# tsnorri/vcf2multialign

Measured on AMD Instinct MI355X. Metric: aligned A2M Gbases/sec, higher is better.
Workload: dtype u8

## Files before the change

### vcf2multialign_amd/csrc/kernels.hpp

```cpp
#pragma once

#include <hip/hip_runtime.h>
#include <stdint.h>

#ifdef V2M_CHECKED_BUILD
__device__ uint32_t v2m_lds_poison_seed;
#endif

namespace v2m {

typedef uint32_t u32;
typedef uint64_t u64;

constexpr int kWave = 64;
typedef u32 vec4u __attribute__((ext_vector_type(4)));
typedef vec4u vec4u_unaligned8 __attribute__((aligned(8)));

#ifdef V2M_CHECKED_BUILD
__device__ __forceinline__ u32 poison_hash(u32 seed, u32 wg, u32 i)
{
	u32 h = seed ^ (wg * 0x9E3779B1u) ^ (i * 0x85EBCA77u);
	h ^= h >> 15; h *= 0x2C1B3C6Du;
	h ^= h >> 12; h *= 0x297A2D39u;
	h ^= h >> 15;
// ... 23 lines not shown
}

__global__ __launch_bounds__(256) void poison_fill_kernel(unsigned char *__restrict__ p, u64 n_bytes, u32 seed, u32 salt)
{
	u64 const n_words = n_bytes / 4;
	for (u64 i = (u64) blockIdx.x * 256 + threadIdx.x; i < n_words; i += (u64) gridDim.x * 256)
		reinterpret_cast<u32 *>(p)[i] = poison_hash(seed, salt, (u32) i);
	if (0 == blockIdx.x && threadIdx.x < (n_bytes & 3))
		p[4 * n_words + threadIdx.x] = (unsigned char) (poison_hash(seed, salt, (u32) n_words) >> (8 * threadIdx.x));
}

#define V2M_POISON_LDS(obj) do { ::v2m::poison_lds_object(obj); asm volatile("s_waitcnt lgkmcnt(0)" ::: "memory"); __syncthreads(); } while (0)
#define V2M_POISON_LDS_RANGE(array, begin, end) ::v2m::poison_lds_words(&(array)[0], (begin), (end))
#else
#define V2M_POISON_LDS(obj) ((void) 0)
#define V2M_POISON_LDS_RANGE(array, begin, end) ((void) 0)
#endif

constexpr int kTileBytes = 16384;
constexpr int kSpliceThreads = 256;
constexpr int kTileChunks = kTileBytes / 16;
constexpr int kChunksPerThread = kTileChunks / kSpliceThreads;
constexpr int kLongPatch = 96;

struct __attribute__((aligned(16))) edge_patch {
	u32 aln_begin;
	u32 aln_end;
	u32 label_begin;
	u32 label_len;
};

struct __attribute__((aligned(8))) edge_span {
	u32 src;
	u32 tgt;
};


constexpr int kTrThreads = 256;

__device__ __forceinline__ u64 shfl_xor_u64(u64 v, int mask)
{
	u32 lo = __shfl_xor((u32) v, mask, kWave);
	u32 hi = __shfl_xor((u32) (v >> 32), mask, kWave);
	return ((u64) hi << 32) | lo;
}

// ... 986 lines not shown
				busy &= busy - 1;
				if (lane == j) {
					for (u64 m = w; m; m &= m - 1) {
						int const b = __builtin_ctzll(m);
						edge_span const sp = spans[wi * 64u + b];
						if (sp.src >= c) {
							out |= 1ULL << b;
							c = sp.tgt;
						}
					}
				}
				c = __shfl(c, j, kWave);
			}
			cur = c;
		} else {
			cur = chunk_max > cur ? chunk_max : cur;
		}
		if (wi < word_end)
			eff_row[wi] = out;
	}
}


struct tile_tables {
	u32 const *edge_begin;
	u32 const *cross_offsets;
	u32 const *cross_edges;
};

template <typename LabelPtr>
__device__ __forceinline__ void fill_patch_bytes(
	unsigned char *tile, u32 tile_base, u32 aln_begin, u32 label_len, LabelPtr label,
	u32 from, u32 to, u32 start, u32 step, char gap)
{
	for (u32 pos = from + start; pos < to; pos += step) {
		u32 const off = pos - aln_begin;
		tile[pos - tile_base] = (off < label_len) ? (unsigned char) label[off] : (unsigned char) gap;
	}
}

constexpr int kCandLds = 512;
constexpr int kLabelLds = 1024;
constexpr int kGroupRowsLds = 16;
constexpr int kEffWordsLds = kCandLds / 64 + 2;
constexpr int kLongQueueLds = 16;

struct cached_patch {
	unsigned short begin_rel;
	unsigned short span;
	unsigned short label_rel;
	unsigned short label_len;
};

struct patch_cache {
	cached_patch patch[kCandLds];
	u64 eff[kGroupRowsLds][kEffWordsLds];
	unsigned char labels[kLabelLds];
	u32 long_queue[kLongQueueLds];
	u32 long_count;
};

struct tile_job {
	u32 tile_base, tile_end;
	u32 cross_begin, n_cross, range_begin, n_range;
	u32 n_lds;
	u32 w0;
};

__device__ __forceinline__ void load_eff_cache(
	patch_cache &pc, tile_job const &job, u64 const *__restrict__ eff, u64 eff_words_per_row, u32 first_row, u32 n_rows, int t)
{
	if (0 == job.n_lds) return;
	u32 const nw = ((job.range_begin + job.n_lds - 1) >> 6) - job.w0 + 1;
	u32 const rows = n_rows < (u32) kGroupRowsLds ? n_rows : (u32) kGroupRowsLds;
	for (u32 i = t; i < rows * nw; i += kSpliceThreads)
		pc.eff[i / nw][i % nw] = eff[(u64) (first_row + i / nw) * eff_words_per_row + job.w0 + i % nw];
}

template <bool kWindow = false>
__device__ __forceinline__ void load_patch_cache(
	patch_cache &pc, tile_job &job, tile_tables const &tt, edge_patch const *__restrict__ patches, char const *__restrict__ labels,
	u64 const *__restrict__ eff, u64 eff_words_per_row, u32 tile, u32 row_begin, u32 n_group_rows, int t, u32 col_base = 0, u32 col_end = 0)
{
	job.tile_base = (kWindow ? col_base : 0u) + tile * (u32) kTileBytes;
	job.tile_end = (kWindow && col_end - job.tile_base < (u32) kTileBytes) ? col_end : job.tile_base + kTileBytes;
	job.cross_begin = tt.cross_offsets[tile];
	job.n_cross = tt.cross_offsets[tile + 1] - job.cross_begin;
	job.range_begin = tt.edge_begin[tile];
	job.n_range = tt.edge_begin[tile + 1] - job.range_begin;
	job.n_lds = job.n_range < (u32) kCandLds ? job.n_range : (u32) kCandLds;
	job.w0 = job.range_begin >> 6;
	if (job.n_lds) {
		u32 const label_base = patches[job.range_begin].label_begin;
		for (u32 i = t; i < job.n_lds; i += kSpliceThreads) {
			edge_patch const p = patches[job.range_begin + i];
			u32 const span = p.aln_end - p.aln_begin, rel = p.label_begin - label_base;
			cached_patch c;
			c.begin_rel = (unsigned short) (p.aln_begin - job.tile_base);
			c.span = span < 0xFFFFu ? (unsigned short) span : (unsigned short) 0xFFFF;
			bool const label_ok = rel + p.label_len <= (u32) kLabelLds;
			c.label_rel = label_ok ? (unsigned short) rel : (unsigned short) 0xFFFF;
			c.label_len = label_ok ? (unsigned short) p.label_len : (unsigned short) 0;
			pc.patch[i] = c;
		}
		edge_patch const last = patches[job.range_begin + job.n_lds - 1];
		u32 const label_span = last.label_begin + last.label_len - label_base;
		u32 const label_len = label_span < (u32) kLabelLds ? label_span : (u32) kLabelLds;
		for (u32 i = t; i < label_len; i += kSpliceThreads)
			pc.labels[i] = (unsigned char) labels[label_base + i];
	}
	load_eff_cache(pc, job, eff, eff_words_per_row, row_begin, n_group_rows, t);
	if (t == 0) pc.long_count = 0;
}

struct tile_patch {
	u32 edge;
	u32 aln_begin;
	u32 from, to;
	u32 label_len;
	u32 label_begin;
	bool in_lds;
};

__device__ __forceinline__ u32 candidate_edge(tile_job const &job, tile_tables const &tt, u32 i)
{
	return (i < job.n_cross) ? tt.cross_edges[job.cross_begin + i] : job.range_begin + (i - job.n_cross);
}

__device__ __forceinline__ bool candidate_in_lds(tile_job const &job, u32 i)
{
	return i >= job.n_cross && i - job.n_cross < job.n_lds;
}

template <bool kWindow = false>
// ... 76 lines not shown
	if (n_long) {
		for (u32 q = t >> 6; q < n_long; q += kSpliceThreads >> 6) {
			edge_patch const p = patches[pc.long_queue[q]];
			u32 const from = p.aln_begin > job.tile_base ? p.aln_begin : job.tile_base;
			u32 const to = p.aln_end < tile_end ? p.aln_end : tile_end;
			fill_patch_bytes(buf, job.tile_base, p.aln_begin, p.label_len, labels + p.label_begin, from, to, t & 63, 64, gap);
		}
		__syncthreads();
		if (t == 0) pc.long_count = 0;
	}
	V2M_POISON_LDS_RANGE(pc.long_queue, 0u, (u32) kLongQueueLds);
}

__device__ __forceinline__ void map_block(u32 b, u32 n_groups, u32 n_tiles, u32 tile_run, u32 &tile, u32 &group)
{
	u32 const per_super = tile_run * n_groups;
	u32 const super = b / per_super, within = b % per_super;
	u32 const t0 = super * tile_run;
	u32 const run = (n_tiles - t0 < tile_run) ? n_tiles - t0 : tile_run;
	group = within / run;
	tile = t0 + within % run;
}

template <bool kNonTemporal, bool kWindow>
__device__ __forceinline__ void splice_aligned_tiles(
	vec4u const *__restrict__ tmpl, u64 const *__restrict__ eff, u64 eff_words_per_row,
	tile_tables tt, edge_patch const *__restrict__ patches, char const *__restrict__ labels,
	char *__restrict__ out, u64 row_pitch, u32 n_rows, u32 rows_per_group, u32 n_groups, u32 n_tiles, u32 tile_run,
	u64 store_limit, char gap, u32 col_base, u32 col_end)
{
	__shared__ vec4u lds[2][kTileChunks];
	__shared__ patch_cache pc;

	int const t = threadIdx.x;
	u32 tile, group;
	map_block(blockIdx.x, n_groups, n_tiles, tile_run, tile, group);
	u32 const row_begin = group * rows_per_group;
	u32 const row_end = (row_begin + rows_per_group < n_rows) ? row_begin + rows_per_group : n_rows;
	V2M_POISON_LDS(lds);
	V2M_POISON_LDS(pc);

	vec4u pristine[kChunksPerThread];
#pragma unroll
	for (int k = 0; k < kChunksPerThread; ++k)
		pristine[k] = tmpl[(u64) tile * kTileChunks + t + kSpliceThreads * k];

	tile_job job;
	load_patch_cache<kWindow>(pc, job, tt, patches, labels, eff, eff_words_per_row, tile, row_begin, row_end - row_begin, t, col_base, col_end);
	u32 const tile_base = job.tile_base;

	for (u32 row = row_begin; row < row_end; ++row) {
		vec4u *const buf = lds[(row - row_begin) & 1];
		u32 const cached_row = (row - row_begin) % (u32) kGroupRowsLds;
		if (row != row_begin && 0 == cached_row)
			load_eff_cache(pc, job, eff, eff_words_per_row, row, row_end - row, t);
#pragma unroll
		for (int k = 0; k < kChunksPerThread; ++k)
			buf[t + kSpliceThreads * k] = pristine[k];
		__syncthreads();

		patch_row_tile<kWindow>((unsigned char *) buf, pc, job, tt, patches, labels, eff + (u64) row * eff_words_per_row, cached_row, t, gap);

		char *const dst = out + (u64) row * row_pitch + (u64) tile * kTileBytes;
#pragma unroll
		for (int k = 0; k < kChunksPerThread; ++k) {
			int const c = t + kSpliceThreads * k;
			if ((kWindow ? (u64) tile * kTileBytes : (u64) tile_base) + (u64) c * 16 < store_limit) {
				vec4u const nv = buf[c];
				if (kNonTemporal)
					__builtin_nontemporal_store(nv, (vec4u *) (dst + c * 16));
				else
					*(vec4u *) (dst + c * 16) = nv;
			}
		}
	}
}

template <bool kNonTemporal>
__global__ __launch_bounds__(kSpliceThreads) void splice_aligned_kernel(
	vec4u const *__restrict__ tmpl, u64 const *__restrict__ eff, u64 eff_words_per_row,
	tile_tables tt, edge_patch const *__restrict__ patches, char const *__restrict__ labels,
	char *__restrict__ out, u64 row_pitch, u32 n_rows, u32 rows_per_group, u32 n_groups, u32 n_tiles, u32 tile_run,
	u64 store_limit , char gap)
{
	splice_aligned_tiles<kNonTemporal, false>(tmpl, eff, eff_words_per_row, tt, patches, labels, out, row_pitch, n_rows, rows_per_group, n_groups,
		n_tiles, tile_run, store_limit, gap, 0u, 0u);
}

template <bool kNonTemporal>
__global__ __launch_bounds__(kSpliceThreads) void splice_aligned_window_kernel(
	vec4u const *__restrict__ tmpl, u64 const *__restrict__ eff, u64 eff_words_per_row,
	tile_tables tt, edge_patch const *__restrict__ patches, char const *__restrict__ labels,
	char *__restrict__ out, u64 row_pitch, u32 n_rows, u32 rows_per_group, u32 n_groups, u32 n_tiles, u32 tile_run,
	u64 store_limit, char gap, u32 col_base, u32 col_end)
{
	splice_aligned_tiles<kNonTemporal, true>(tmpl, eff, eff_words_per_row, tt, patches, labels, out, row_pitch, n_rows, rows_per_group, n_groups,
		n_tiles, tile_run, store_limit, gap, col_base, col_end);
}


__device__ __forceinline__ u32 zero_bytes_mask(u32 x)
{
	return ~(((x & 0x7F7F7F7Fu) + 0x7F7F7F7Fu) | x | 0x7F7F7F7Fu);
}

__device__ __forceinline__ u32 wave_inclusive_scan_u32(u32 v)
{
	v += (u32) __builtin_amdgcn_update_dpp(0, (int) v, 0x111, 0xf, 0xf, false);
	v += (u32) __builtin_amdgcn_update_dpp(0, (int) v, 0x112, 0xf, 0xf, false);
	v += (u32) __builtin_amdgcn_update_dpp(0, (int) v, 0x114, 0xf, 0xf, false);
	v += (u32) __builtin_amdgcn_update_dpp(0, (int) v, 0x118, 0xf, 0xf, false);
	v += (u32) __builtin_amdgcn_update_dpp(0, (int) v, 0x142, 0xa, 0xf, false);
	v += (u32) __builtin_amdgcn_update_dpp(0, (int) v, 0x143, 0xc, 0xf, false);
	return v;
}

template <int kN>
__device__ __forceinline__ void wave_inclusive_scan_u32_lockstep(u32 (&v)[kN])
{
// ... 484 lines not shown
	__syncthreads();
	for (u32 base = 0; base < n_tiles; base += 256) {
		u32 const i = base + t;
		u32 const mine = i < n_tiles ? row[i] : 0;
		u32 const incl = wave_inclusive_scan_u32(mine);
		if (lane == 63) wave_sums[wave] = incl;
		__syncthreads();
		u32 before = carry_s, total = 0;
#pragma unroll
		for (int wv = 0; wv < 4; ++wv) {
			u32 const ws = wave_sums[wv];
			if (wv < wave) before += ws;
			total += ws;
		}
		if (i < n_tiles) row[i] = before + incl - mine;
		__syncthreads();
		if (t == 0) carry_s += total;
		__syncthreads();
	}
	if (t == 0) row_lengths[blockIdx.x] = carry_s;
}


__global__ __launch_bounds__(kSpliceThreads) void probe_write_kernel(char *__restrict__ out, u64 pitch, u32 n_groups)
{
	u32 const tile = blockIdx.x / n_groups, group = blockIdx.x % n_groups;
	vec4u const v = {0, 0, 0, 0};
	for (u32 r = 0; r < 16; ++r) {
		char *const dst = out + (u64) (group * 16 + r) * pitch + (u64) tile * kTileBytes;
#pragma unroll
		for (int k = 0; k < kChunksPerThread; ++k)
			__builtin_nontemporal_store(v, (vec4u *) (dst + (threadIdx.x + kSpliceThreads * k) * 16));
	}
}


__host__ __device__ __forceinline__ u64 mix64(u64 z)
{
	z ^= z >> 30; z *= 0xBF58476D1CE4E5B9ULL;
	z ^= z >> 27; z *= 0x94D049BB133111EBULL;
	z ^= z >> 31;
	return z;
}

constexpr u64 kGolden = 0x9E3779B97F4A7C15ULL;

__global__ __launch_bounds__(256) void checksum_rows_kernel(
	char const *__restrict__ rows, u64 row_pitch, u64 const *__restrict__ lengths, u64 fixed_length,
	u64 words_per_block, unsigned long long *__restrict__ sums)
{
	u32 const row = blockIdx.y;
	u64 const len = lengths ? lengths[row] : fixed_length;
	u64 const n_words = (len + 7) / 8;
	u64 const w_begin = (u64) blockIdx.x * words_per_block;
	u64 w_end = w_begin + words_per_block;
// ... 22 lines not shown
```

### vcf2multialign_amd/csrc/v2m_hip.hip

```cpp

#include <hip/hip_runtime.h>

#include <algorithm>
#include <atomic>
#include <chrono>
#include <condition_variable>
#include <cstdarg>
#include <cstdio>
#include <cstdlib>
#include <cstring>
#include <memory>
#include <mutex>
#include <string>
#include <thread>
#include <utility>
#include <vector>

#include <type_traits>

#include "../../include/v2m_hip.h"
#include "kernels.hpp"
#include "founder_kernels.hpp"
#include "bgzf_kernels.hpp"

// ... 100 lines not shown


struct held_ring_state {
	std::mutex mutex;
	std::condition_variable released;
};

struct v2m_row_hold {
	pinned_buf host;
	hipEvent_t copied{};
	uint64_t outstanding{};
	held_ring_state *ring{};
};


struct word_range { u64 restart, lo, hi, stride; };

struct row_view {
	u64 begin{}, end{};
	u64 max_unaligned{};
	u32 n_tiles{};
	dev_buf d_template, d_template0;
	bool has_template0{};
	dev_buf d_edge_begin, d_cross_offsets, d_cross_edges;
	word_range words{};
	u64 length() const { return end - begin; }
};


struct v2m_ctx {
	int device{};
	u32 n_cus{256};
	hipStream_t stream{};
	hipStream_t copy_stream{};
	std::string err;

	bool profiling{};
	std::vector<event_pair> events[V2M_KERNEL_COUNT];
	std::vector<event_pair> free_events;

	bool has_graph{};
	u64 n_nodes{}, n_edges{}, ref_len{}, aligned_len{}, label_bytes{};
	bool has_nul_byte{};
	std::vector<u32> h_csum;
	std::vector<u32> h_tgt_prefix_max;
	dev_buf d_ref, d_ref_pos, d_aln_pos, d_spans, d_patches, d_labels, d_overlappable;
	dev_buf d_ovl_rank, d_blocker_masks;
	std::vector<u32> h_aln_pos, h_tile_edge_begin, h_cross_offsets, h_cross_edges;
// ... 71 lines not shown
	{
		if (!ctx->profiling) return;
		if (!ctx->free_events.empty()) { ev = ctx->free_events.back(); ctx->free_events.pop_back(); }
		else if (hipSuccess != hipEventCreate(&ev.begin) || hipSuccess != hipEventCreate(&ev.end)) return;
		active = (hipSuccess == hipEventRecord(ev.begin, ctx->stream));
	}
	~timed_launch()
	{
		if (!active) return;
		(void) hipEventRecord(ev.end, ctx->stream);
		ctx->events[kernel].push_back(ev);
	}
};


template <typename T>
int upload_vec(v2m_ctx *ctx, dev_buf &dst, std::vector<T> const &src, size_t min_bytes = 16)
{
	size_t const bytes(std::max(src.size() * sizeof(T), min_bytes));
	V2M_HIP_TRY(ctx, dst.ensure(bytes));
	if (!src.empty())
		V2M_HIP_TRY(ctx, hipMemcpyAsync(dst.p, src.data(), src.size() * sizeof(T), hipMemcpyHostToDevice, ctx->stream));
	return V2M_OK;
}


struct scoped_events {
	std::vector<hipEvent_t> ev;
	~scoped_events() { for (auto e : ev) (void) hipEventDestroy(e); }
	hipError_t create(std::size_t n)
	{
		for (std::size_t i(0); i < n; ++i) {
			hipEvent_t e{};
			hipError_t const st(hipEventCreate(&e));
			if (hipSuccess != st) return st;
			ev.push_back(e);
		}
		return hipSuccess;
	}
	hipEvent_t operator[](std::size_t i) const { return ev[i]; }
};

struct scoped_profiling_off {
	v2m_ctx *ctx;
	bool was;
	explicit scoped_profiling_off(v2m_ctx *c) : ctx(c), was(c->profiling) { c->profiling = false; }
// ... 380 lines not shown
			out.seg_copy[n] = copy;
			++n;
			prev = node;
		}
	});
	std::vector<row_error> errors(n_rows);
	unsigned const n_threads(out.n_segments >= (u64(1) << 20) ? unsigned(std::min<u64>(n_rows, 8)) : 1u);
	if (n_threads <= 1) {
		for (u64 r(row_begin); r < row_end; ++r) { fill_row(r, errors[r - row_begin]); if (V2M_OK != errors[r - row_begin].code) break; }
	}
	else {
		std::atomic<u64> next(row_begin);
		auto const work([&] { for (u64 r; (r = next.fetch_add(1)) < row_end;) fill_row(r, errors[r - row_begin]); });
		std::vector<std::thread> pool;
		for (unsigned t(1); t < n_threads; ++t) pool.emplace_back(work);
		work();
		for (auto &t : pool) t.join();
	}
	for (auto const &e : errors) if (V2M_OK != e.code) return fail(ctx, e.code, "%s", e.text.c_str());
	return V2M_OK;
}


int forced_store_mode(bool unaligned)
{
	if (unaligned) {
		char const *const e = std::getenv("V2M_UNALIGNED_STORE");
		if (e && 0 == std::strcmp(e, "plain")) return 0;
		if (e && 0 == std::strcmp(e, "nt")) return 1;
		return -1;
	}
	char const *e = std::getenv("V2M_NT_STORES");
	if (!(e && *e)) return -1;
	return std::atoi(e) != 0 ? 1 : 0;
}

u32 rows_per_group_for(u64 n_rows)
{
	char const *e = std::getenv("V2M_ROWS_PER_GROUP");
	int const v((e && *e) ? std::atoi(e) : 0);
	if (v > 0) return u32(std::min(v, 256));
	return u32(std::min<u64>(32, std::max<u64>(1, n_rows)));
}


int expand_reference(v2m_ctx *ctx, row_view const &v, dev_buf &dst, char gap)
{
	u64 const n_chunks(u64(v.n_tiles) * v2m::kTileChunks);
	V2M_HIP_TRY(ctx, dst.ensure(n_chunks * 16));
	{
		timed_launch tl(ctx, V2M_KERNEL_TEMPLATE);
		hipLaunchKernelGGL(v2m::expand_reference_row_kernel, dim3(unsigned((n_chunks + 255) / 256)), dim3(256), 0, ctx->stream,
			ctx->d_ref.as<char>(), ctx->d_ref_pos.as<u32>(), ctx->d_aln_pos.as<u32>(), u32(ctx->n_nodes), u32(v.end), n_chunks, dst.as<uint4>(), gap, u32(v.begin));
	}
// ... 80 lines not shown
	u64 n_blocks;
};

u32 tile_run_for(u32 n_tiles)
{
	char const *e = std::getenv("V2M_TILE_RUN");
	int const v((e && *e) ? std::atoi(e) : 0);
	u32 const run(v > 0 ? u32(v) : 64u);
	return std::max<u32>(1, std::min(run, n_tiles));
}

int make_grid(v2m_ctx *ctx, u64 n_rows, splice_grid &g)
{
	g.rows_per_group = rows_per_group_for(n_rows);
	g.n_groups = u32((n_rows + g.rows_per_group - 1) / g.rows_per_group);
	g.n_blocks = u64(ctx->view().n_tiles) * g.n_groups;
	g.tile_run = tile_run_for(ctx->view().n_tiles);
	if (g.n_blocks > 0x7FFFFFFFull)
		return fail(ctx, V2M_ERR_UNSUPPORTED, "splice grid too large (%llu workgroups); use smaller batches", (unsigned long long) g.n_blocks);
	return V2M_OK;
}


template <typename F>
int store_flavour_launch(v2m_ctx *ctx, bool unaligned, u64 n_rows, u64 bytes, F const &launch)
{
	int &slot(unaligned ? ctx->unaligned_store_mode : ctx->store_mode);
	int mode(forced_store_mode(unaligned));
	if (mode < 0) mode = slot;
	if (mode < 0 && bytes >= (u64(1) << 30)) {
		scoped_events ev;
		V2M_HIP_TRY(ctx, ev.create(5));
		V2M_HIP_TRY(ctx, hipEventRecord(ev[0], ctx->stream));
		for (int i(0); i < 4; ++i) {
			launch(0 == (i & 1));
			V2M_HIP_TRY(ctx, hipEventRecord(ev[i + 1], ctx->stream));
		}
		V2M_HIP_TRY(ctx, hipStreamSynchronize(ctx->stream));
		float t[4];
		for (int i(0); i < 4; ++i) V2M_HIP_TRY(ctx, hipEventElapsedTime(&t[i], ev[i], ev[i + 1]));
		float const nt_ms(std::min(t[0], t[2])), plain_ms(std::min(t[1], t[3]));
		slot = nt_ms <= plain_ms ? 1 : 0;
		char buf[160];
		std::snprintf(buf, sizeof(buf), "%s splice stores: %s (calibrated on %llu rows: nontemporal %.3f ms, plain %.3f ms)",
			unaligned ? "unaligned" : "aligned", slot ? "nontemporal" : "plain", (unsigned long long) n_rows, nt_ms, plain_ms);
		if (unaligned && ctx->info.size() > 2000) ctx->info.clear();
		if (!ctx->info.empty()) ctx->info += "; ";
		ctx->info += buf;
		mode = slot;
	}
	if (mode < 0) mode = 1;
	{
		timed_launch tl(ctx, unaligned ? V2M_KERNEL_SPLICE_UNALIGNED : V2M_KERNEL_SPLICE_ALIGNED);
		launch(0 != mode);
	}
	V2M_HIP_TRY(ctx, hipGetLastError());
	return V2M_OK;
}


int splice_aligned_slice(v2m_ctx *ctx, v2m_row_batch const *rows, u64 row_begin, u64 row_end, char *d_out, u64 row_pitch)
{
	u64 const n_rows(row_end - row_begin);
	if (0 == n_rows || 0 == ctx->aligned_len) return V2M_OK;
	if (int const rc = resolve_slice(ctx, rows, row_begin, row_end)) return rc;

	row_view const &v(ctx->view());
	splice_grid g;
	if (int const rc = make_grid(ctx, n_rows, g)) return rc;
	v2m::tile_tables const tt{v.d_edge_begin.as<u32>(), v.d_cross_offsets.as<u32>(), v.d_cross_edges.as<u32>()};
	u64 const store_limit((v.length() + 15) & ~u64(15));
	auto const launch([&](bool nt) {
		auto const go([&](auto kernel, auto... window) {
			hipLaunchKernelGGL(kernel, dim3(unsigned(g.n_blocks)), dim3(v2m::kSpliceThreads), 0, ctx->stream,
				v.d_template.as<v2m::vec4u>(), ctx->d_eff.as<u64>() - v.words.restart, v.words.stride, tt, ctx->d_patches.as<v2m::edge_patch>(), ctx->d_labels.as<char>(),
				d_out, row_pitch, u32(n_rows), g.rows_per_group, g.n_groups, v.n_tiles, g.tile_run, store_limit, '-', window...);
		});
		if (ctx->windowed) {
			if (nt) go(v2m::splice_aligned_window_kernel<true>, u32(v.begin), u32(v.end));
			else go(v2m::splice_aligned_window_kernel<false>, u32(v.begin), u32(v.end));
		}
		else if (nt) go(v2m::splice_aligned_kernel<true>);
		else go(v2m::splice_aligned_kernel<false>);
	});
	return store_flavour_launch(ctx, false, n_rows, n_rows * v.length(), launch);
}


int splice_unaligned_slice(v2m_ctx *ctx, v2m_row_batch const *rows, u64 row_begin, u64 row_end, char *d_out, u64 row_pitch)
{
	u64 const n_rows(row_end - row_begin);
	if (0 == n_rows) return V2M_OK;
	V2M_HIP_TRY(ctx, ctx->d_row_lengths.ensure(n_rows * sizeof(u64)));
	if (0 == ctx->aligned_len) {
		V2M_HIP_TRY(ctx, hipMemsetAsync(ctx->d_row_lengths.p, 0, n_rows * sizeof(u64), ctx->stream));
		return V2M_OK;
	}
	row_view &v(ctx->view());
	if (!v.has_template0) {
		if (int const rc = expand_reference(ctx, v, v.d_template0, 0)) return rc;
		v.has_template0 = true;
	}
	if (int const rc = resolve_slice(ctx, rows, row_begin, row_end)) return rc;

	splice_grid g;
	if (int const rc = make_grid(ctx, n_rows, g)) return rc;
	V2M_HIP_TRY(ctx, ctx->d_tile_counts.ensure(n_rows * v.n_tiles * sizeof(u32)));
	bool const windowed(ctx->windowed);
	v2m::tile_tables const tt{v.d_edge_begin.as<u32>(), v.d_cross_offsets.as<u32>(), v.d_cross_edges.as<u32>()};
	u64 const *const d_eff(ctx->d_eff.as<u64>() - v.words.restart);
	{
		char const *const ce(std::getenv("V2M_COUNT_ROWS_PER_GROUP"));
		u32 const count_rows(u32(std::min<u64>(std::max<u64>(1, n_rows), (ce && *ce && std::atoi(ce) > 0) ? u64(std::min(std::atoi(ce), int(v2m::kCountRowsMax))) : u64(v2m::kCountRowsMax))));
		u32 const count_groups(u32((n_rows + count_rows - 1) / count_rows));
		timed_launch tl(ctx, V2M_KERNEL_UNALIGNED_COUNT);
		auto const count([&](auto kernel, auto... window) {
			hipLaunchKernelGGL(kernel, dim3(unsigned(u64(v.n_tiles) * count_groups)), dim3(v2m::kSpliceThreads), 0, ctx->stream,
				v.d_template0.as<v2m::vec4u>(), d_eff, v.words.stride, tt, ctx->d_patches.as<v2m::edge_patch>(), ctx->d_labels.as<char>(),
				ctx->d_tile_counts.as<u32>(), v.n_tiles, u32(n_rows), count_rows, count_groups, g.tile_run, window...);
		});
		if (windowed) count(v2m::count_unaligned_window_kernel, u32(v.begin), u32(v.end));
		else count(v2m::count_unaligned_kernel);
		hipLaunchKernelGGL(v2m::scan_tile_counts_kernel, dim3(unsigned(n_rows)), dim3(256), 0, ctx->stream,
			ctx->d_tile_counts.as<u32>(), v.n_tiles, ctx->d_row_lengths.as<u64>());
	}
	auto const launch([&](bool nt) {
		auto const go([&](auto kernel, auto... window) {
			hipLaunchKernelGGL(kernel, dim3(unsigned(g.n_blocks)), dim3(v2m::kSpliceThreads), 0, ctx->stream,
				v.d_template0.as<v2m::vec4u>(), d_eff, v.words.stride, tt, ctx->d_patches.as<v2m::edge_patch>(), ctx->d_labels.as<char>(),
				ctx->d_tile_counts.as<u32>(), v.n_tiles, d_out, row_pitch, u32(n_rows), g.rows_per_group, g.n_groups, g.tile_run, window...);
		});
		if (windowed) {
			if (nt) go(v2m::splice_unaligned_window_kernel<true>, u32(v.begin), u32(v.end));
			else go(v2m::splice_unaligned_window_kernel<false>, u32(v.begin), u32(v.end));
			return;
		}
#ifdef V2M_TUNING_BUILD
		static int const flavour([] { char const *const e(std::getenv("V2M_UNALIGNED_KERNEL")); return !e ? 0 : 0 == std::strcmp(e, "wave") ? 1 : 0 == std::strcmp(e, "shared64") ? 2 : 0; }());
		if (1 == flavour) { if (nt) go(v2m::splice_unaligned_per_wave_kernel<true>); else go(v2m::splice_unaligned_per_wave_kernel<false>); return; }
		if (2 == flavour) { if (nt) go(v2m::splice_unaligned_kernel<true, 64>); else go(v2m::splice_unaligned_kernel<false, 64>); return; }
#endif
		if (nt) go(v2m::splice_unaligned_kernel<true>);
		else go(v2m::splice_unaligned_kernel<false>);
	});
	return store_flavour_launch(ctx, true, n_rows, n_rows * (windowed ? v.length() : ctx->ref_len), launch);
}


int check_batch(v2m_ctx *ctx, v2m_row_batch const *rows, u32 flags)
{
	if (!ctx) return V2M_ERR_INVALID_ARGUMENT;
	if (!rows) return fail(ctx, V2M_ERR_INVALID_ARGUMENT, "rows is NULL");
	if (flags & ~(V2M_SPLICE_UNALIGNED | V2M_SPLICE_BGZF)) return fail(ctx, V2M_ERR_INVALID_ARGUMENT, "unknown flags 0x%x", flags);
	if (!ctx->has_graph) return fail(ctx, V2M_ERR_STATE, "no graph uploaded");
	if (rows->n_rows && !rows->copy_index && !rows->cut_offsets) return fail(ctx, V2M_ERR_INVALID_ARGUMENT, "rows->copy_index is NULL");
	if (rows->cut_offsets && rows->cut_offsets[rows->n_rows] && (!rows->cut_nodes || !rows->cut_copies))
		return fail(ctx, V2M_ERR_INVALID_ARGUMENT, "cut arrays are NULL");
	if (rows->n_rows >= 0xFFFFFFFFull) return fail(ctx, V2M_ERR_UNSUPPORTED, "too many rows in one batch");
	if (ctx->d_by_edge.p) { ctx->d_by_edge.reset(); ctx->by_edge_valid = false; }
	if ((flags & V2M_SPLICE_UNALIGNED) && ctx->has_nul_byte)
		return fail(ctx, V2M_ERR_UNSUPPORTED, "the reference sequence or an ALT label holds a NUL byte, which the unaligned kernels use as their padding marker; aligned mode keeps such bytes");
	return V2M_OK;
}


struct slice_plan { u64 pitch, rows_per_slice, n_slices, slot_bytes; };

slice_plan plan_slices(v2m_ctx const *ctx, u64 n_rows, bool unaligned, u64 max_rows_per_slice = ~u64(0))
// ... 601 lines not shown
	ctx->n_nodes = N; ctx->n_edges = E; ctx->ref_len = ref_len; ctx->aligned_len = L; ctx->label_bytes = label_total;
	V2M_HIP_TRY(ctx, ctx->d_ref.ensure(std::max<u64>(ref_len, 16)));
	if (ref_len) V2M_HIP_TRY(ctx, hipMemcpyAsync(ctx->d_ref.p, ref_seq, ref_len, hipMemcpyHostToDevice, ctx->stream));
	V2M_HIP_TRY(ctx, ctx->d_labels.ensure(std::max<u64>(label_total, 16)));
	if (label_total) V2M_HIP_TRY(ctx, hipMemcpyAsync(ctx->d_labels.p, g->alt_edge_label_bytes, label_total, hipMemcpyHostToDevice, ctx->stream));
	if (int const rc = upload_vec(ctx, ctx->d_ref_pos, ref_pos)) return rc;
	if (int const rc = upload_vec(ctx, ctx->d_aln_pos, aln_pos)) return rc;
	if (int const rc = upload_vec(ctx, ctx->d_spans, spans)) return rc;
	if (int const rc = upload_vec(ctx, ctx->d_patches, patches)) return rc;
	if (int const rc = upload_vec(ctx, ctx->d_overlappable, overlappable)) return rc;
	if (int const rc = upload_vec(ctx, ctx->d_ovl_rank, ovl_rank)) return rc;
	if (int const rc = upload_vec(ctx, ctx->d_blocker_masks, blocker_masks)) return rc;

	row_view &v(ctx->whole);
	v.begin = 0;
	v.end = L;
	v.max_unaligned = ref_len + label_total;
	v.n_tiles = n_tiles;
	v.has_template0 = false;
	v.words = {0, 0, (E + 63) / 64, (((E + 63) / 64) + 15) & ~u64(15)};
	if (int const rc = upload_vec(ctx, v.d_edge_begin, tile_edge_begin)) return rc;
	if (int const rc = upload_vec(ctx, v.d_cross_offsets, cross_offsets)) return rc;
	if (int const rc = upload_vec(ctx, v.d_cross_edges, cross_edges)) return rc;
	if (int const rc = expand_reference(ctx, v, v.d_template, '-')) return rc;

	ctx->d_paths = nullptr;
	ctx->by_edge_valid = false;
	ctx->path_rows = ctx->path_cols = ctx->path_pitch = 0;
	if (g->paths_by_chrom_copy_and_edge) {
		size_t const bytes(g->path_rows / 64 * g->path_cols * sizeof(u64));
		V2M_HIP_TRY(ctx, ctx->owned_paths.ensure(std::max<size_t>(bytes, 16)));
		if (bytes) V2M_HIP_TRY(ctx, hipMemcpyAsync(ctx->owned_paths.p, g->paths_by_chrom_copy_and_edge, bytes, hipMemcpyHostToDevice, ctx->stream));
		ctx->d_paths = ctx->owned_paths.as<u64>();
		ctx->path_rows = g->path_rows;
		ctx->path_cols = g->path_cols;
		ctx->path_pitch = g->path_rows / 64;
	}
	V2M_HIP_TRY(ctx, hipStreamSynchronize(ctx->stream));

	ctx->has_nul_byte = (ref_len && std::memchr(ref_seq, 0, ref_len)) || (label_total && std::memchr(g->alt_edge_label_bytes, 0, label_total));
	ctx->h_csum = std::move(csum);
	ctx->h_tgt_prefix_max = std::move(tgt_prefix_max);
	ctx->h_aln_pos = std::move(aln_pos);
	ctx->h_patches = std::move(patches);
	ctx->h_overlappable = std::move(overlappable);
	ctx->h_tile_edge_begin = std::move(tile_edge_begin);
// ... 171 lines not shown
	u32 const e_hi(edge_begin[n_tiles]);
	u64 e_lo(0), hi(e_hi);
	while (e_lo < hi) {
		u64 const mid((e_lo + hi) / 2);
		if (ctx->h_aln_pos[ctx->h_tgt_prefix_max[mid + 1]] > col_begin) hi = mid; else e_lo = mid + 1;
	}
	row_view &w(ctx->window);
	u64 restart(0), lo(0), word_hi(0);
	if (e_lo < e_hi) {
		lo = e_lo / 64;
		word_hi = (u64(e_hi) + 63) / 64;
		restart = lo;
		while (restart > 0 && (ctx->h_overlappable[restart] & 1)) --restart;
	}
	w.words = {restart, lo, word_hi, (word_hi - restart + 15) & ~u64(15)};
	w.begin = col_begin;
	w.end = col_end;
	w.max_unaligned = W;
	w.n_tiles = n_tiles;
	w.has_template0 = false;
	if (int const rc = upload_vec(ctx, w.d_edge_begin, edge_begin)) return rc;
	if (int const rc = upload_vec(ctx, w.d_cross_offsets, cross_offsets)) return rc;
	if (int const rc = upload_vec(ctx, w.d_cross_edges, cross_edges)) return rc;
	if (int const rc = expand_reference(ctx, w, w.d_template, '-')) return rc;
	V2M_HIP_TRY(ctx, hipStreamSynchronize(ctx->stream));
	ctx->windowed = true;
	return V2M_OK;
}



namespace {

int pbwt_check_state(v2m_ctx *ctx, uint64_t n_copies, uint64_t n_chunks, const uint32_t *start_order, int max_copies)
{
	if (0 == n_copies || n_copies > u64(max_copies)) return fail(ctx, V2M_ERR_UNSUPPORTED, "this GPU chunk walk holds at most %d chromosome copies (got %llu)", max_copies, (unsigned long long) n_copies);
	if (n_copies > ctx->path_cols) return fail(ctx, V2M_ERR_INVALID_ARGUMENT, "the bound path matrix has %llu copies, %llu asked for", (unsigned long long) ctx->path_cols, (unsigned long long) n_copies);
	if (ctx->path_cols > u64(max_copies)) return fail(ctx, V2M_ERR_UNSUPPORTED, "this GPU chunk walk reads edge columns of at most %d copies; the bound path matrix has %llu columns", max_copies, (unsigned long long) ctx->path_cols);
	if (ctx->n_edges >= 0x7FFFFFF0ull) return fail(ctx, V2M_ERR_UNSUPPORTED, "the GPU chunk walk keeps edge indices in 31 bits (the graph has %llu edges)", (unsigned long long) ctx->n_edges);
	for (u64 i(0), n(n_chunks * n_copies); i < n; ++i)
		if (start_order[i] >= n_copies) return fail(ctx, V2M_ERR_INVALID_ARGUMENT, "start_order[%llu] = %u is not a chromosome copy (%llu copies)", (unsigned long long) i, start_order[i], (unsigned long long) n_copies);
	return V2M_OK;
}

int edge_major_paths(v2m_ctx *ctx, u64 const **d_by_edge_out)
{
// ... 291 lines not shown
	});
}

void v2m_row_release(v2m_row_hold *hold)
{
	if (!hold) return;
	std::lock_guard<std::mutex> const lock(hold->ring->mutex);
	if (hold->outstanding && 0 == --hold->outstanding) hold->ring->released.notify_all();
}




namespace {

int probe_output(v2m_ctx *ctx, void *p, u64 pitch, u32 n_groups, float &ms_out)
{
	scoped_events ev;
	V2M_HIP_TRY(ctx, ev.create(2));
	u32 const n_tiles(u32(pitch / v2m::kTileBytes));
	ms_out = 1e30f;
	for (int rep(0); rep < 3; ++rep) {
		V2M_HIP_TRY(ctx, hipEventRecord(ev[0], ctx->stream));
		hipLaunchKernelGGL(v2m::probe_write_kernel, dim3(n_tiles * n_groups), dim3(v2m::kSpliceThreads), 0, ctx->stream, static_cast<char *>(p), pitch, n_groups);
		V2M_HIP_TRY(ctx, hipEventRecord(ev[1], ctx->stream));
		V2M_HIP_TRY(ctx, hipEventSynchronize(ev[1]));
		float t(0);
		V2M_HIP_TRY(ctx, hipEventElapsedTime(&t, ev[0], ev[1]));
		if (rep) ms_out = std::min(ms_out, t);
	}
	return V2M_OK;
}

}

int v2m_alloc_output(v2m_ctx *ctx, uint64_t bytes, int candidates, void **d_out)
{
	if (!ctx) return V2M_ERR_INVALID_ARGUMENT;
	if (!d_out || 0 == bytes) return fail(ctx, V2M_ERR_INVALID_ARGUMENT, "bad v2m_alloc_output arguments");
	*d_out = nullptr;
	V2M_HIP_TRY(ctx, hipSetDevice(ctx->device));

	u32 const n_groups(32);
	u64 const pitch((bytes / (n_groups * 16)) & ~u64(v2m::kTileBytes - 1));
	bool const can_probe(pitch >= u64(64) * v2m::kTileBytes);
	auto const note([&](std::string const &text) {
		if (ctx->info.size() > 2000) ctx->info.clear();
// ... 375 lines not shown
```

Baseline: 6874.

## Use buffer stores with cache-policy flavours and precomputed tile descriptors in aligned splice

Aligned splice stores now go through raw buffer stores with selectable cache-policy bits (nt, sc1_nt, sc0_sc1_nt, plain), and the runtime calibration picks the fastest of these flavours. The buffer resource range replaces the per-chunk store_limit bounds check. Per-tile metadata and label extents are precomputed on the host into a tile_desc array, so the patch, label and eff-cache loads are issued up front as unrolled buffer loads. The eff cache refill is moved after patching, which overlaps it with the stores. This adds a host-side table and a wider calibration sweep over large outputs. It relies on out-of-range buffer accesses being dropped.

Measured after the change: 6850, median of 2. No clear change (-0.3%).

```diff
diff --git a/vcf2multialign_amd/csrc/kernels.hpp b/vcf2multialign_amd/csrc/kernels.hpp
--- a/vcf2multialign_amd/csrc/kernels.hpp
+++ b/vcf2multialign_amd/csrc/kernels.hpp
@@ -69,6 +69,26 @@
 constexpr int kTileChunks = kTileBytes / 16;
 constexpr int kChunksPerThread = kTileChunks / kSpliceThreads;
 constexpr int kLongPatch = 96;
+
+enum class store_flavour : int { plain = 0, nt = 1, sc1 = 2, sc1_nt = 3, sc0_sc1 = 4, sc0_sc1_nt = 5, flat_nt = 6 };
+
+__host__ __device__ constexpr int store_aux(store_flavour f)
+{
+	return store_flavour::nt == f ? 2 : store_flavour::sc1 == f ? 16 : store_flavour::sc1_nt == f ? 18
+		: store_flavour::sc0_sc1 == f ? 17 : store_flavour::sc0_sc1_nt == f ? 19 : 0;
+}
+
+__device__ __forceinline__ __amdgpu_buffer_rsrc_t tile_store_rsrc(char *p, u32 bytes)
+{
+	return __builtin_amdgcn_make_buffer_rsrc(p,  0, (int) bytes, 0x00020000);
+}
+
+template <store_flavour kFlavour>
+__device__ __forceinline__ void store_tile_chunk(__amdgpu_buffer_rsrc_t rsrc, u32 off, u32 __attribute__((ext_vector_type(4))) value)
+{
+	static_assert(store_flavour::flat_nt != kFlavour, "flat_nt is not a buffer store");
+	__builtin_amdgcn_raw_buffer_store_b128(value, rsrc, (int) off, 0, store_aux(kFlavour));
+}
 
 struct __attribute__((aligned(16))) edge_patch {
 	u32 aln_begin;
@@ -1101,10 +1121,12 @@
 }
 
 
+struct tile_desc;
 struct tile_tables {
 	u32 const *edge_begin;
 	u32 const *cross_offsets;
 	u32 const *cross_edges;
+	tile_desc const *desc;
 };
 
 template <typename LabelPtr>
@@ -1139,6 +1161,13 @@
 	u32 long_count;
 };
 
+struct __attribute__((aligned(32))) tile_desc {
+	u32 range_begin, n_range;
+	u32 cross_begin, n_cross;
+	u32 label_base, label_bytes;
+	u32 reserved[2];
+};
+
 struct tile_job {
 	u32 tile_base, tile_end;
 	u32 cross_begin, n_cross, range_begin, n_range;
@@ -1163,32 +1192,53 @@
 {
 	job.tile_base = (kWindow ? col_base : 0u) + tile * (u32) kTileBytes;
 	job.tile_end = (kWindow && col_end - job.tile_base < (u32) kTileBytes) ? col_end : job.tile_base + kTileBytes;
-	job.cross_begin = tt.cross_offsets[tile];
-	job.n_cross = tt.cross_offsets[tile + 1] - job.cross_begin;
-	job.range_begin = tt.edge_begin[tile];
-	job.n_range = tt.edge_begin[tile + 1] - job.range_begin;
+	tile_desc const d = tt.desc[tile];
+	job.cross_begin = d.cross_begin;
+	job.n_cross = d.n_cross;
+	job.range_begin = d.range_begin;
+	job.n_range = d.n_range;
 	job.n_lds = job.n_range < (u32) kCandLds ? job.n_range : (u32) kCandLds;
 	job.w0 = job.range_begin >> 6;
-	if (job.n_lds) {
-		u32 const label_base = patches[job.range_begin].label_begin;
-		for (u32 i = t; i < job.n_lds; i += kSpliceThreads) {
-			edge_patch const p = patches[job.range_begin + i];
-			u32 const span = p.aln_end - p.aln_begin, rel = p.label_begin - label_base;
-			cached_patch c;
-			c.begin_rel = (unsigned short) (p.aln_begin - job.tile_base);
-			c.span = span < 0xFFFFu ? (unsigned short) span : (unsigned short) 0xFFFF;
-			bool const label_ok = rel + p.label_len <= (u32) kLabelLds;
-			c.label_rel = label_ok ? (unsigned short) rel : (unsigned short) 0xFFFF;
-			c.label_len = label_ok ? (unsigned short) p.label_len : (unsigned short) 0;
-			pc.patch[i] = c;
-		}
-		edge_patch const last = patches[job.range_begin + job.n_lds - 1];
-		u32 const label_span = last.label_begin + last.label_len - label_base;
-		u32 const label_len = label_span < (u32) kLabelLds ? label_span : (u32) kLabelLds;
-		for (u32 i = t; i < label_len; i += kSpliceThreads)
-			pc.labels[i] = (unsigned char) labels[label_base + i];
-	}
-	load_eff_cache(pc, job, eff, eff_words_per_row, row_begin, n_group_rows, t);
+
+	constexpr int kPatchLoads = kCandLds / kSpliceThreads, kLabelLoads = kLabelLds / kSpliceThreads;
+	static_assert(kPatchLoads * kSpliceThreads == kCandLds && kLabelLoads * kSpliceThreads == kLabelLds, "whole rounds of the workgroup");
+	static_assert(kGroupRowsLds * kEffWordsLds <= kSpliceThreads, "one effective-edge word per thread");
+	__amdgpu_buffer_rsrc_t const patch_rsrc = __builtin_amdgcn_make_buffer_rsrc(
+		const_cast<edge_patch *>(patches + job.range_begin), 0, (int) (job.n_lds * (u32) sizeof(edge_patch)), 0x00020000);
+	__amdgpu_buffer_rsrc_t const label_rsrc = __builtin_amdgcn_make_buffer_rsrc(const_cast<char *>(labels + d.label_base), 0, (int) d.label_bytes, 0x00020000);
+	vec4u pv[kPatchLoads];
+	unsigned char lb[kLabelLoads];
+#pragma unroll
+	for (int k = 0; k < kPatchLoads; ++k)
+		pv[k] = __builtin_amdgcn_raw_buffer_load_b128(patch_rsrc, (int) ((t + kSpliceThreads * k) * sizeof(edge_patch)), 0, 0);
+#pragma unroll
+	for (int k = 0; k < kLabelLoads; ++k)
+		lb[k] = __builtin_amdgcn_raw_buffer_load_b8(label_rsrc, t + kSpliceThreads * k, 0, 0);
+	u32 const nw = job.n_lds ? ((job.range_begin + job.n_lds - 1) >> 6) - job.w0 + 1 : 0u;
+	u32 const eff_rows = n_group_rows < (u32) kGroupRowsLds ? n_group_rows : (u32) kGroupRowsLds;
+	bool const has_eff = (u32) t < eff_rows * nw;
+	u32 const eff_r = has_eff ? (u32) t / nw : 0u, eff_w = has_eff ? (u32) t % nw : 0u;
+	u64 eff_word = 0;
+	if (has_eff) eff_word = eff[(u64) (row_begin + eff_r) * eff_words_per_row + job.w0 + eff_w];
+
+#pragma unroll
+	for (int k = 0; k < kPatchLoads; ++k) {
+		u32 const i = t + kSpliceThreads * k;
+		if (i >= job.n_lds) continue;
+		edge_patch const p{pv[k].x, pv[k].y, pv[k].z, pv[k].w};
+		u32 const span = p.aln_end - p.aln_begin, rel = p.label_begin - d.label_base;
+		cached_patch c;
+		c.begin_rel = (unsigned short) (p.aln_begin - job.tile_base);
+		c.span = span < 0xFFFFu ? (unsigned short) span : (unsigned short) 0xFFFF;
+		bool const label_ok = rel + p.label_len <= (u32) kLabelLds;
+		c.label_rel = label_ok ? (unsigned short) rel : (unsigned short) 0xFFFF;
+		c.label_len = label_ok ? (unsigned short) p.label_len : (unsigned short) 0;
+		pc.patch[i] = c;
+	}
+#pragma unroll
+	for (int k = 0; k < kLabelLoads; ++k)
+		if ((u32) (t + kSpliceThreads * k) < d.label_bytes) pc.labels[t + kSpliceThreads * k] = lb[k];
+	if (has_eff) pc.eff[eff_r][eff_w] = eff_word;
 	if (t == 0) pc.long_count = 0;
 }
 
@@ -1311,7 +1361,7 @@
 	tile = t0 + within % run;
 }
 
-template <bool kNonTemporal, bool kWindow>
+template <store_flavour kFlavour, bool kWindow>
 __device__ __forceinline__ void splice_aligned_tiles(
 	vec4u const *__restrict__ tmpl, u64 const *__restrict__ eff, u64 eff_words_per_row,
 	tile_tables tt, edge_patch const *__restrict__ patches, char const *__restrict__ labels,
@@ -1336,13 +1386,12 @@
 
 	tile_job job;
 	load_patch_cache<kWindow>(pc, job, tt, patches, labels, eff, eff_words_per_row, tile, row_begin, row_end - row_begin, t, col_base, col_end);
-	u32 const tile_base = job.tile_base;
+	u64 const tile_off = (u64) tile * kTileBytes;
+	u32 const tile_bytes = store_limit <= tile_off ? 0u : store_limit - tile_off < (u64) kTileBytes ? (u32) (store_limit - tile_off) : (u32) kTileBytes;
 
 	for (u32 row = row_begin; row < row_end; ++row) {
 		vec4u *const buf = lds[(row - row_begin) & 1];
 		u32 const cached_row = (row - row_begin) % (u32) kGroupRowsLds;
-		if (row != row_begin && 0 == cached_row)
-			load_eff_cache(pc, job, eff, eff_words_per_row, row, row_end - row, t);
 #pragma unroll
 		for (int k = 0; k < kChunksPerThread; ++k)
 			buf[t + kSpliceThreads * k] = pristine[k];
@@ -1350,40 +1399,37 @@
 
 		patch_row_tile<kWindow>((unsigned char *) buf, pc, job, tt, patches, labels, eff + (u64) row * eff_words_per_row, cached_row, t, gap);
 
-		char *const dst = out + (u64) row * row_pitch + (u64) tile * kTileBytes;
+		if (cached_row + 1 == (u32) kGroupRowsLds && row + 1 < row_end)
+			load_eff_cache(pc, job, eff, eff_words_per_row, row + 1, row_end - (row + 1), t);
+
+		__amdgpu_buffer_rsrc_t const rsrc = tile_store_rsrc(out + (u64) row * row_pitch + tile_off, tile_bytes);
 #pragma unroll
 		for (int k = 0; k < kChunksPerThread; ++k) {
 			int const c = t + kSpliceThreads * k;
-			if ((kWindow ? (u64) tile * kTileBytes : (u64) tile_base) + (u64) c * 16 < store_limit) {
-				vec4u const nv = buf[c];
-				if (kNonTemporal)
-					__builtin_nontemporal_store(nv, (vec4u *) (dst + c * 16));
-				else
-					*(vec4u *) (dst + c * 16) = nv;
-			}
-		}
-	}
-}
-
-template <bool kNonTemporal>
+			store_tile_chunk<kFlavour>(rsrc, (u32) c * 16, buf[c]);
+		}
+	}
+}
+
+template <store_flavour kFlavour>
 __global__ __launch_bounds__(kSpliceThreads) void splice_aligned_kernel(
 	vec4u const *__restrict__ tmpl, u64 const *__restrict__ eff, u64 eff_words_per_row,
 	tile_tables tt, edge_patch const *__restrict__ patches, char const *__restrict__ labels,
 	char *__restrict__ out, u64 row_pitch, u32 n_rows, u32 rows_per_group, u32 n_groups, u32 n_tiles, u32 tile_run,
 	u64 store_limit , char gap)
 {
-	splice_aligned_tiles<kNonTemporal, false>(tmpl, eff, eff_words_per_row, tt, patches, labels, out, row_pitch, n_rows, rows_per_group, n_groups,
+	splice_aligned_tiles<kFlavour, false>(tmpl, eff, eff_words_per_row, tt, patches, labels, out, row_pitch, n_rows, rows_per_group, n_groups,
 		n_tiles, tile_run, store_limit, gap, 0u, 0u);
 }
 
-template <bool kNonTemporal>
+template <store_flavour kFlavour>
 __global__ __launch_bounds__(kSpliceThreads) void splice_aligned_window_kernel(
 	vec4u const *__restrict__ tmpl, u64 const *__restrict__ eff, u64 eff_words_per_row,
 	tile_tables tt, edge_patch const *__restrict__ patches, char const *__restrict__ labels,
 	char *__restrict__ out, u64 row_pitch, u32 n_rows, u32 rows_per_group, u32 n_groups, u32 n_tiles, u32 tile_run,
 	u64 store_limit, char gap, u32 col_base, u32 col_end)
 {
-	splice_aligned_tiles<kNonTemporal, true>(tmpl, eff, eff_words_per_row, tt, patches, labels, out, row_pitch, n_rows, rows_per_group, n_groups,
+	splice_aligned_tiles<kFlavour, true>(tmpl, eff, eff_words_per_row, tt, patches, labels, out, row_pitch, n_rows, rows_per_group, n_groups,
 		n_tiles, tile_run, store_limit, gap, col_base, col_end);
 }
 
@@ -1914,15 +1960,23 @@
 }
 
 
-__global__ __launch_bounds__(kSpliceThreads) void probe_write_kernel(char *__restrict__ out, u64 pitch, u32 n_groups)
+template <store_flavour kFlavour>
+__global__ __launch_bounds__(kSpliceThreads) void probe_write_kernel(char *__restrict__ out, u64 pitch, u32 n_groups, u32 fill)
 {
 	u32 const tile = blockIdx.x / n_groups, group = blockIdx.x % n_groups;
-	vec4u const v = {0, 0, 0, 0};
+	vec4u const v = {fill, fill * (threadIdx.x | 1u), fill * (tile | 1u), fill ^ (fill >> 7)};
 	for (u32 r = 0; r < 16; ++r) {
 		char *const dst = out + (u64) (group * 16 + r) * pitch + (u64) tile * kTileBytes;
-#pragma unroll
-		for (int k = 0; k < kChunksPerThread; ++k)
-			__builtin_nontemporal_store(v, (vec4u *) (dst + (threadIdx.x + kSpliceThreads * k) * 16));
+		if constexpr (store_flavour::flat_nt == kFlavour) {
+#pragma unroll
+			for (int k = 0; k < kChunksPerThread; ++k)
+				__builtin_nontemporal_store(v, (vec4u *) (dst + (threadIdx.x + kSpliceThreads * k) * 16));
+		} else {
+			__amdgpu_buffer_rsrc_t const rsrc = tile_store_rsrc(dst, (u32) kTileBytes);
+#pragma unroll
+			for (int k = 0; k < kChunksPerThread; ++k)
+				store_tile_chunk<kFlavour>(rsrc, (threadIdx.x + kSpliceThreads * k) * 16u, v);
+		}
 	}
 }
 
diff --git a/vcf2multialign_amd/csrc/v2m_hip.hip b/vcf2multialign_amd/csrc/v2m_hip.hip
--- a/vcf2multialign_amd/csrc/v2m_hip.hip
+++ b/vcf2multialign_amd/csrc/v2m_hip.hip
@@ -146,8 +146,9 @@
 	u32 n_tiles{};
 	dev_buf d_template, d_template0;
 	bool has_template0{};
-	dev_buf d_edge_begin, d_cross_offsets, d_cross_edges;
+	dev_buf d_edge_begin, d_cross_offsets, d_cross_edges, d_tile_desc;
 	word_range words{};
+	v2m::tile_tables tables() const { return {d_edge_begin.as<u32>(), d_cross_offsets.as<u32>(), d_cross_edges.as<u32>(), d_tile_desc.as<v2m::tile_desc>()}; }
 	u64 length() const { return end - begin; }
 };
 
@@ -265,6 +266,22 @@
 	if (!src.empty())
 		V2M_HIP_TRY(ctx, hipMemcpyAsync(dst.p, src.data(), src.size() * sizeof(T), hipMemcpyHostToDevice, ctx->stream));
 	return V2M_OK;
+}
+
+
+std::vector<v2m::tile_desc> make_tile_descs(std::vector<v2m::edge_patch> const &patches, std::vector<u32> const &edge_begin, std::vector<u32> const &cross_offsets, u32 n_tiles)
+{
+	std::vector<v2m::tile_desc> descs(n_tiles);
+	for (u32 t(0); t < n_tiles; ++t) {
+		v2m::tile_desc &d(descs[t]);
+		d = {edge_begin[t], edge_begin[t + 1] - edge_begin[t], cross_offsets[t], cross_offsets[t + 1] - cross_offsets[t], 0, 0, {0, 0}};
+		u32 const n_lds(std::min<u32>(d.n_range, v2m::kCandLds));
+		if (!n_lds) continue;
+		v2m::edge_patch const &last(patches[d.range_begin + n_lds - 1]);
+		d.label_base = patches[d.range_begin].label_begin;
+		d.label_bytes = std::min<u32>(last.label_begin + last.label_len - d.label_base, v2m::kLabelLds);
+	}
+	return descs;
 }
 
 
@@ -691,6 +708,12 @@
 }
 
 
+struct flavour_name { int mode; char const *name; };
+constexpr flavour_name kUnalignedFlavours[] = {{1, "nontemporal"}, {0, "plain"}};
+constexpr flavour_name kAlignedFlavours[] = {
+	{int(v2m::store_flavour::nt), "nt"}, {int(v2m::store_flavour::sc1_nt), "sc1_nt"},
+	{int(v2m::store_flavour::sc0_sc1_nt), "sc0_sc1_nt"}, {int(v2m::store_flavour::plain), "plain"}};
+
 int forced_store_mode(bool unaligned)
 {
 	if (unaligned) {
@@ -699,6 +722,9 @@
 		if (e && 0 == std::strcmp(e, "nt")) return 1;
 		return -1;
 	}
+	if (char const *const name = std::getenv("V2M_ALIGNED_STORE"))
+		for (auto const &f : kAlignedFlavours)
+			if (0 == std::strcmp(name, f.name)) return f.mode;
 	char const *e = std::getenv("V2M_NT_STORES");
 	if (!(e && *e)) return -1;
 	return std::atoi(e) != 0 ? 1 : 0;
@@ -825,37 +851,48 @@
 }
 
 
-template <typename F>
-int store_flavour_launch(v2m_ctx *ctx, bool unaligned, u64 n_rows, u64 bytes, F const &launch)
+template <std::size_t kN, typename F>
+int store_flavour_launch(v2m_ctx *ctx, bool unaligned, flavour_name const (&flavours)[kN], u64 n_rows, u64 bytes, F const &launch)
 {
 	int &slot(unaligned ? ctx->unaligned_store_mode : ctx->store_mode);
 	int mode(forced_store_mode(unaligned));
 	if (mode < 0) mode = slot;
 	if (mode < 0 && bytes >= (u64(1) << 30)) {
 		scoped_events ev;
-		V2M_HIP_TRY(ctx, ev.create(5));
+		V2M_HIP_TRY(ctx, ev.create(2 * kN + 1));
 		V2M_HIP_TRY(ctx, hipEventRecord(ev[0], ctx->stream));
-		for (int i(0); i < 4; ++i) {
-			launch(0 == (i & 1));
+		for (std::size_t i(0); i < 2 * kN; ++i) {
+			launch(flavours[i % kN].mode);
 			V2M_HIP_TRY(ctx, hipEventRecord(ev[i + 1], ctx->stream));
 		}
 		V2M_HIP_TRY(ctx, hipStreamSynchronize(ctx->stream));
-		float t[4];
-		for (int i(0); i < 4; ++i) V2M_HIP_TRY(ctx, hipEventElapsedTime(&t[i], ev[i], ev[i + 1]));
-		float const nt_ms(std::min(t[0], t[2])), plain_ms(std::min(t[1], t[3]));
-		slot = nt_ms <= plain_ms ? 1 : 0;
-		char buf[160];
-		std::snprintf(buf, sizeof(buf), "%s splice stores: %s (calibrated on %llu rows: nontemporal %.3f ms, plain %.3f ms)",
-			unaligned ? "unaligned" : "aligned", slot ? "nontemporal" : "plain", (unsigned long long) n_rows, nt_ms, plain_ms);
+		float ms[kN];
+		std::size_t best(0);
+		for (std::size_t i(0); i < kN; ++i) {
+			float a(0), b(0);
+			V2M_HIP_TRY(ctx, hipEventElapsedTime(&a, ev[i], ev[i + 1]));
+			V2M_HIP_TRY(ctx, hipEventElapsedTime(&b, ev[kN + i], ev[kN + i + 1]));
+			ms[i] = std::min(a, b);
+			if (ms[i] < ms[best]) best = i;
+		}
+		slot = flavours[best].mode;
+		char buf[96];
+		std::snprintf(buf, sizeof(buf), "%s splice stores: %s (calibrated on %llu rows:", unaligned ? "unaligned" : "aligned", flavours[best].name, (unsigned long long) n_rows);
+		std::string text(buf);
+		for (std::size_t i(0); i < kN; ++i) {
+			std::snprintf(buf, sizeof(buf), "%s %s %.3f ms", i ? "," : "", flavours[i].name, ms[i]);
+			text += buf;
+		}
+		text += ")";
 		if (unaligned && ctx->info.size() > 2000) ctx->info.clear();
 		if (!ctx->info.empty()) ctx->info += "; ";
-		ctx->info += buf;
+		ctx->info += text;
 		mode = slot;
 	}
 	if (mode < 0) mode = 1;
 	{
 		timed_launch tl(ctx, unaligned ? V2M_KERNEL_SPLICE_UNALIGNED : V2M_KERNEL_SPLICE_ALIGNED);
-		launch(0 != mode);
+		launch(mode);
 	}
 	V2M_HIP_TRY(ctx, hipGetLastError());
 	return V2M_OK;
@@ -871,22 +908,28 @@
 	row_view const &v(ctx->view());
 	splice_grid g;
 	if (int const rc = make_grid(ctx, n_rows, g)) return rc;
-	v2m::tile_tables const tt{v.d_edge_begin.as<u32>(), v.d_cross_offsets.as<u32>(), v.d_cross_edges.as<u32>()};
+	v2m::tile_tables const tt(v.tables());
 	u64 const store_limit((v.length() + 15) & ~u64(15));
-	auto const launch([&](bool nt) {
+	auto const launch([&](int mode) {
 		auto const go([&](auto kernel, auto... window) {
 			hipLaunchKernelGGL(kernel, dim3(unsigned(g.n_blocks)), dim3(v2m::kSpliceThreads), 0, ctx->stream,
 				v.d_template.as<v2m::vec4u>(), ctx->d_eff.as<u64>() - v.words.restart, v.words.stride, tt, ctx->d_patches.as<v2m::edge_patch>(), ctx->d_labels.as<char>(),
 				d_out, row_pitch, u32(n_rows), g.rows_per_group, g.n_groups, v.n_tiles, g.tile_run, store_limit, '-', window...);
 		});
-		if (ctx->windowed) {
-			if (nt) go(v2m::splice_aligned_window_kernel<true>, u32(v.begin), u32(v.end));
-			else go(v2m::splice_aligned_window_kernel<false>, u32(v.begin), u32(v.end));
-		}
-		else if (nt) go(v2m::splice_aligned_kernel<true>);
-		else go(v2m::splice_aligned_kernel<false>);
+		auto const with([&](auto flavour) {
+			constexpr v2m::store_flavour kF(decltype(flavour)::value);
+			if (ctx->windowed) go(v2m::splice_aligned_window_kernel<kF>, u32(v.begin), u32(v.end));
+			else go(v2m::splice_aligned_kernel<kF>);
+		});
+		using sf = v2m::store_flavour;
+		switch (sf(mode)) {
+			case sf::plain: with(std::integral_constant<sf, sf::plain>{}); break;
+			case sf::sc1_nt: with(std::integral_constant<sf, sf::sc1_nt>{}); break;
+			case sf::sc0_sc1_nt: with(std::integral_constant<sf, sf::sc0_sc1_nt>{}); break;
+			default: with(std::integral_constant<sf, sf::nt>{}); break;
+		}
 	});
-	return store_flavour_launch(ctx, false, n_rows, n_rows * v.length(), launch);
+	return store_flavour_launch(ctx, false, kAlignedFlavours, n_rows, n_rows * v.length(), launch);
 }
 
 
@@ -910,7 +953,7 @@
 	if (int const rc = make_grid(ctx, n_rows, g)) return rc;
 	V2M_HIP_TRY(ctx, ctx->d_tile_counts.ensure(n_rows * v.n_tiles * sizeof(u32)));
 	bool const windowed(ctx->windowed);
-	v2m::tile_tables const tt{v.d_edge_begin.as<u32>(), v.d_cross_offsets.as<u32>(), v.d_cross_edges.as<u32>()};
+	v2m::tile_tables const tt(v.tables());
 	u64 const *const d_eff(ctx->d_eff.as<u64>() - v.words.restart);
 	{
 		char const *const ce(std::getenv("V2M_COUNT_ROWS_PER_GROUP"));
@@ -927,7 +970,8 @@
 		hipLaunchKernelGGL(v2m::scan_tile_counts_kernel, dim3(unsigned(n_rows)), dim3(256), 0, ctx->stream,
 			ctx->d_tile_counts.as<u32>(), v.n_tiles, ctx->d_row_lengths.as<u64>());
 	}
-	auto const launch([&](bool nt) {
+	auto const launch([&](int mode) {
+		bool const nt(0 != mode);
 		auto const go([&](auto kernel, auto... window) {
 			hipLaunchKernelGGL(kernel, dim3(unsigned(g.n_blocks)), dim3(v2m::kSpliceThreads), 0, ctx->stream,
 				v.d_template0.as<v2m::vec4u>(), d_eff, v.words.stride, tt, ctx->d_patches.as<v2m::edge_patch>(), ctx->d_labels.as<char>(),
@@ -946,7 +990,7 @@
 		if (nt) go(v2m::splice_unaligned_kernel<true>);
 		else go(v2m::splice_unaligned_kernel<false>);
 	});
-	return store_flavour_launch(ctx, true, n_rows, n_rows * (windowed ? v.length() : ctx->ref_len), launch);
+	return store_flavour_launch(ctx, true, kUnalignedFlavours, n_rows, n_rows * (windowed ? v.length() : ctx->ref_len), launch);
 }
 
 
@@ -1594,6 +1638,7 @@
 	if (int const rc = upload_vec(ctx, v.d_edge_begin, tile_edge_begin)) return rc;
 	if (int const rc = upload_vec(ctx, v.d_cross_offsets, cross_offsets)) return rc;
 	if (int const rc = upload_vec(ctx, v.d_cross_edges, cross_edges)) return rc;
+	if (int const rc = upload_vec(ctx, v.d_tile_desc, make_tile_descs(patches, tile_edge_begin, cross_offsets, n_tiles), sizeof(v2m::tile_desc))) return rc;
 	if (int const rc = expand_reference(ctx, v, v.d_template, '-')) return rc;
 
 	ctx->d_paths = nullptr;
@@ -1811,6 +1856,7 @@
 	if (int const rc = upload_vec(ctx, w.d_edge_begin, edge_begin)) return rc;
 	if (int const rc = upload_vec(ctx, w.d_cross_offsets, cross_offsets)) return rc;
 	if (int const rc = upload_vec(ctx, w.d_cross_edges, cross_edges)) return rc;
+	if (int const rc = upload_vec(ctx, w.d_tile_desc, make_tile_descs(patches, edge_begin, cross_offsets, n_tiles), sizeof(v2m::tile_desc))) return rc;
 	if (int const rc = expand_reference(ctx, w, w.d_template, '-')) return rc;
 	V2M_HIP_TRY(ctx, hipStreamSynchronize(ctx->stream));
 	ctx->windowed = true;
@@ -2148,7 +2194,7 @@
 	ms_out = 1e30f;
 	for (int rep(0); rep < 3; ++rep) {
 		V2M_HIP_TRY(ctx, hipEventRecord(ev[0], ctx->stream));
-		hipLaunchKernelGGL(v2m::probe_write_kernel, dim3(n_tiles * n_groups), dim3(v2m::kSpliceThreads), 0, ctx->stream, static_cast<char *>(p), pitch, n_groups);
+		hipLaunchKernelGGL(v2m::probe_write_kernel<v2m::store_flavour::flat_nt>, dim3(n_tiles * n_groups), dim3(v2m::kSpliceThreads), 0, ctx->stream, static_cast<char *>(p), pitch, n_groups, 0u);
 		V2M_HIP_TRY(ctx, hipEventRecord(ev[1], ctx->stream));
 		V2M_HIP_TRY(ctx, hipEventSynchronize(ev[1]));
 		float t(0);
```
